# chaiyujin/sdfa-2019

Measured on AMD Instinct MI355X. Metric: animation frames/s/node (10 s@16 kHz clips); max|Δdgrad| vs CPU ref, higher is better.
Workload: dtype f32

## Files before the change

### sdfa-2019_amd/csrc/api_core.cpp

```cpp
#include "../../include/sdfa_stream.h"
#include "host.h"

#include <climits>
#include <cstdio>
#include <cstring>
#include <string>

static thread_local std::string g_err;

int sdfa_failv(int code, const char *fmt, va_list ap) {
    char buf[512];
    vsnprintf(buf, sizeof buf, fmt, ap);
    g_err = buf;
    return code;
}

int sdfa_fail(int code, const char *fmt, ...) {
    va_list ap;
    va_start(ap, fmt);
    sdfa_failv(code, fmt, ap);
    va_end(ap);
    return code;
}

thread_local int g_sdfa_mel_fft_radix4 = 0;
thread_local int g_sdfa_gather_plain_order = 0;
thread_local int g_sdfa_frontend_two_kernel = 0;
thread_local int g_sdfa_frontend_stream_block = 0;
thread_local int g_sdfa_frontend_stream_slots = 0;
thread_local int g_sdfa_frontend_stream_spin_max = 0;
thread_local int g_sdfa_frontend_stream_phases = 0;
thread_local int g_sdfa_frontend_t_major = 0;
extern thread_local int g_sdfa_gemm_variant;
thread_local int g_sdfa_freq_lstm_shape = 0;
thread_local int g_sdfa_pca_lds = 0;
thread_local int g_sdfa_pca_fp32 = 0;
thread_local int g_sdfa_conv_fp32 = 0;
thread_local int g_sdfa_time_lstm_split = 0;
thread_local int g_sdfa_time_lstm_fuse_x = 0;
thread_local int g_sdfa_time_lstm_handoff = 0;
thread_local int g_sdfa_time_lstm_timeout_us = 0;
thread_local int g_sdfa_share_gx0_off = 0;
thread_local int g_sdfa_encoder_dedup_off = 0;
thread_local int g_sdfa_share_hash_bits = 0;
thread_local int g_sdfa_freq_proj_tail = 0;
thread_local int g_sdfa_attn_unfused = 0;

extern "C" {

int sdfa_abi_version(void) { return SDFA_ABI_VERSION; }
int sdfa_stream_abi_version(void) { return SDFA_STREAM_ABI_VERSION; }
const char *sdfa_last_error(void) { return g_err.c_str(); }

int sdfa_debug_set_option(const char *name, int value) {
    struct Option { const char *name; int *var; int lo = INT_MIN, hi = INT_MAX; const char *accepts = nullptr; };
    thread_local const Option options[] = {
        {"attn_unfused", &g_sdfa_attn_unfused},
        {"share_gx0_off", &g_sdfa_share_gx0_off},
        {"encoder_dedup_off", &g_sdfa_encoder_dedup_off},
        {"share_hash_bits", &g_sdfa_share_hash_bits, 0, 32, "0 (the whole hash) or 1..32 low bits"},
        {"freq_proj_tail", &g_sdfa_freq_proj_tail, 0, 2, "0 (rule), 1 (never) or 2 (always)"},
        {"frontend_two_kernel", &g_sdfa_frontend_two_kernel},
        {"frontend_stream_phases", &g_sdfa_frontend_stream_phases},
        {"frontend_stream_spin_max", &g_sdfa_frontend_stream_spin_max, 0, INT_MAX, "0 (default) or a positive poll count"},
        {"frontend_stream_block", &g_sdfa_frontend_stream_block, 0, 256, "0 (default) or 1..256 frames"},
        {"frontend_stream_slots", &g_sdfa_frontend_stream_slots, 0, 256, "0 (default) or 1..256 workgroups per block"},
        {"gather_plain_order", &g_sdfa_gather_plain_order},
        {"mel_fft_radix4", &g_sdfa_mel_fft_radix4},
        {"frontend_t_major", &g_sdfa_frontend_t_major},
        {"time_lstm_timeout_us", &g_sdfa_time_lstm_timeout_us},
        {"time_lstm_handoff", &g_sdfa_time_lstm_handoff},
        {"time_lstm_split", &g_sdfa_time_lstm_split},
        {"time_lstm_fuse_x", &g_sdfa_time_lstm_fuse_x, 0, 3, "0 (rule), 1 (never), 2 or 3 (always, 32- / 64-frame tiles)"},
        {"gemm_variant", &g_sdfa_gemm_variant},
        {"freq_lstm_shape", &g_sdfa_freq_lstm_shape},
        {"pca_lds", &g_sdfa_pca_lds},
        {"conv_fp32", &g_sdfa_conv_fp32},
        {"pca_fp32", &g_sdfa_pca_fp32},
    };
    for (const Option &o : options)
        if (name && !strcmp(name, o.name)) {
            if (value < o.lo || value > o.hi) return sdfa_fail(SDFA_EINVAL, "%s: %s", o.name, o.accepts);
            *o.var = value;
            return SDFA_OK;
        }
    return sdfa_fail(SDFA_EINVAL, "unknown option '%s'", name ? name : "(null)");
}

}
```

### sdfa-2019_amd/csrc/api_forward.cpp

```cpp
#include "common.h"
#include "host.h"
#include "kernels.h"
#include "model.h"

#include <algorithm>

extern thread_local int g_sdfa_gemm_variant, g_sdfa_freq_lstm_shape, g_sdfa_pca_lds, g_sdfa_pca_fp32, g_sdfa_conv_fp32, g_sdfa_share_gx0_off, g_sdfa_attn_unfused, g_sdfa_encoder_dedup_off,
    g_sdfa_freq_proj_tail, g_sdfa_share_hash_bits;

namespace {

constexpr int64_t CT_WORDS = 2048, CT_FLAGS = 16, ST_WORDS = SDFA_WS_STATUS_BYTES / 4;

struct Ws {
    int64_t P1, X3, HF, Z, GX, H0, H1, KP, QC, QP, ZK, SH, ZU, total;
    int64_t TRUNK, A0, A1, COEF;
    int64_t CT_FREQ, CT_PCA, CT_FLAG;
};

Ws layout(int64_t Nc, bool keep) {
    const int64_t Mc = 64 * Nc;
    Ws w{};
    int64_t o = 0;
    auto take = [&](int64_t n) { int64_t r = o; o += round_up(n, 64); return r; };
    take(ST_WORDS);
    if (keep) {
        w.P1 = take(2048 * Mc); w.X3 = take(2048 * Mc); w.HF = take((int64_t)HF_SLAB_ROWS * 4 * Mc); w.Z = take(256 * Mc);
        w.GX = take(2048 * Mc); w.H0 = take(512 * Mc); w.H1 = take(512 * Mc); w.KP = take(128 * Mc);
    } else {
        const int64_t A = take(2048 * Mc);
        const int64_t B = take(2048 * Mc);
        w.HF = take((int64_t)HF_SLAB_ROWS * 4 * Mc);
        w.P1 = A; w.GX = A;
        w.X3 = B; w.Z = B; w.H0 = B + 256 * Mc; w.H1 = B + 768 * Mc; w.KP = B + 1280 * Mc;
    }
    w.QC = take(512 * Nc); w.QP = take(128 * Nc); w.ZK = take(512 * Nc);
    const int64_t R = take(2560 * Nc);
    w.TRUNK = R; w.A0 = R + 512 * Nc; w.A1 = R + 1024 * Nc; w.COEF = R + 1280 * Nc;
    w.SH = take(sdfa_share_table_words(Nc) + 111);
    w.ZU = keep ? take(256 * Mc) : w.P1;
    const int64_t CT = take(CT_WORDS);
    w.CT_FREQ = CT; w.CT_PCA = CT + 1; w.CT_FLAG = CT + CT_FLAGS;
    w.total = o;
    return w;
}

int64_t capacity(int64_t bytes, bool keep) {
    const int64_t per128 = layout(128, keep).total * 4;
    int64_t nc = (bytes / per128 + 2) * 128;
    while (nc > 0 && layout(nc, keep).total * 4 > bytes) nc -= 128;
    return nc;
}

struct Prof {
    const sdfa_model *m;
    hipStream_t s;
    hipEvent_t pending = nullptr;
    void begin(const char *stage) {
        if (!m->profile) return;
        sdfa_model::Ev e; e.stage = stage;
        (void)hipEventCreate(&e.a); (void)hipEventCreate(&e.b);
// ... 64 lines not shown
    case SDFA_PREC_BF16X3_ATTENTION: return stage == STAGE_ATTENTION ? 3 : 0;
    case SDFA_PREC_BF16X6: return 6;
    case SDFA_PREC_BF16X3: return 3;
    case SDFA_PREC_BF16: return 1;
    default: return 0;
    }
}

int sdfa_model_set_precision(sdfa_model *m, int mode) {
    if (!m) return sdfa_fail(SDFA_EINVAL, "null model");
    if (mode < SDFA_PREC_FP32 || mode > SDFA_PREC_BF16X6) return sdfa_fail(SDFA_EINVAL, "unknown precision mode %d", mode);
    m->precision = mode;
    return SDFA_OK;
}

int sdfa_model_precision(const sdfa_model *m) { return m ? m->precision : SDFA_EINVAL; }

int sdfa_model_set_reserved_cus(sdfa_model *m, int k) {
    if (!m) return sdfa_fail(SDFA_EINVAL, "null model");
    if (k < 0 || k > 128) return sdfa_fail(SDFA_EINVAL, "reserved_cus must be in [0, 128], got %d", k);
    m->reserved_cus.store(k);
    return SDFA_OK;
}

static int encoder_impl(const sdfa_model *m, const float *d_audio_feat, int64_t n_frames, const int32_t *d_frame_clip,
                        const int64_t *d_frame_start, int hop, float *d_z, float *d_align, void *d_workspace,
                        int64_t workspace_bytes, void *stream) {
    if (!m || !m->finalized) return sdfa_fail(SDFA_ESTATE, "encoder_forward: model not finalised");
    if (n_frames == 0) return SDFA_OK;
    if (!d_audio_feat || !d_z || !d_workspace || n_frames < 0) return sdfa_fail(SDFA_EINVAL, "encoder_forward: bad argument");
    if (((uintptr_t)d_workspace | (uintptr_t)d_audio_feat | (uintptr_t)d_z) & 15) return sdfa_fail(SDFA_EINVAL, "encoder_forward: pointers must be 16-byte aligned");
    if ((uintptr_t)d_align & 3) return sdfa_fail(SDFA_EINVAL, "encoder_forward: d_align must be 4-byte aligned");
    const int64_t cap = capacity(workspace_bytes, m->keep);
    if (cap < 128) return sdfa_fail(SDFA_ENOSPACE, "encoder_forward: workspace of %lld bytes holds no 128-frame chunk", (long long)workspace_bytes);
    hipStream_t s = (hipStream_t)stream;
    Prof pf{m, s};
    float *ws = (float *)d_workspace;
    for (int64_t f0 = 0; f0 < n_frames; f0 += cap) {
        const int64_t N = std::min(cap, n_frames - f0);
        const int64_t Nc = round_up(N, 128), Mc = 64 * Nc;
        const Ws w = layout(Nc, m->keep);
        ConvArgs ca{};
        ca.audio_feat = d_audio_feat + f0 * (64 * 128 * 3); ca.N = N; ca.Nc = Nc; ca.Mc = Mc;
        ca.w1 = m->w1; ca.b1 = m->b1; ca.s1 = m->s1; ca.t1 = m->t1; ca.P1 = ws + w.P1;
        ca.w2 = m->w2; ca.b2 = m->b2; ca.s2 = m->s2; ca.t2 = m->t2;
        ca.w3 = m->w3; ca.b3 = m->b3; ca.s3 = m->s3; ca.t3 = m->t3; ca.X3 = ws + w.X3;
        const bool table = d_frame_clip != nullptr;
        const bool share = table || (!m->keep && !g_sdfa_encoder_dedup_off);
        const int64_t *d_ulimit = nullptr;
        int32_t *col_to_u = nullptr;
        bool split_tail = false;
        int64_t fat_grid = 0;
        const int64_t *d_qfull = nullptr;
        if (share) {
            ShareArgs sa{};
            sa.N = N; sa.Nc = Nc; sa.Mc = Mc;
            sdfa_share_carve(sa, reinterpret_cast<int32_t *>(ws + w.SH));
            split_tail = !m->keep && stage_terms(m, STAGE_BODY) == 0 && g_sdfa_gemm_variant == 0 && Mc / 256 >= 512 && g_sdfa_freq_proj_tail != 1;
            if (split_tail) {
                fat_grid = sdfa_fat_grid(256, Mc, sdfa_cu_count(), m->reserved_cus.load());
                sa.fat_grid = (int)fat_grid; sa.tail_mode = g_sdfa_freq_proj_tail;
            }
            pf.begin("share_map");
            if (table) {
                sa.frame_clip = d_frame_clip + f0; sa.frame_start = d_frame_start + f0; sa.hop = hop;
                sa.t_lo = 6; sa.t_hi = 58;
                HIP_TRY(sdfa_launch_share_map(sa, s));
            } else {
                sa.feat = ca.audio_feat;
                sa.hash = reinterpret_cast<uint64_t *>(ws + w.HF);
                sa.group_slots = sdfa_share_group_slots(N);
                sa.group_key = sa.hash + Mc; sa.group_first = reinterpret_cast<uint32_t *>(sa.group_key + sa.group_slots);
                sa.hash_bits = g_sdfa_share_hash_bits;
                HIP_TRY(sdfa_launch_share_map_content(sa, s));
            }
            pf.end();
            d_ulimit = sa.counts + 1; d_qfull = sa.counts + 2; col_to_u = sa.col_to_u;
            ca.col_src = sa.col_src; ca.col_limit = d_ulimit;
        }
        const int conv_terms = g_sdfa_conv_fp32 ? 0 : stage_terms(m, STAGE_BODY);
        if (m->keep && conv_terms) {
            pf.begin("conv1"); HIP_TRY(sdfa_launch_conv1(ca, s)); pf.end();
            ca.wb = m->cv_wb; ca.terms = conv_terms;
            pf.begin("conv23"); HIP_TRY(sdfa_launch_conv123(ca, s)); pf.end();
        } else if (m->keep) {
            pf.begin("conv1"); HIP_TRY(sdfa_launch_conv1(ca, s)); pf.end();
            pf.begin("conv23"); HIP_TRY(sdfa_launch_conv23(ca, s)); pf.end();
        } else {
            ca.wb = m->cv_wb; ca.terms = conv_terms;
            pf.begin("conv23"); HIP_TRY(sdfa_launch_conv123(ca, s)); pf.end();
        }

        const int fl_terms = stage_terms(m, STAGE_BODY);
        FreqLstmArgs fa{ws + w.X3, m->fl_w, m->fl_b, ws + w.HF, Mc, d_ulimit, m->fl_wb, fl_terms, reinterpret_cast<int *>(ws + w.CT_FREQ),
                        g_sdfa_freq_lstm_shape ? g_sdfa_freq_lstm_shape : (fl_terms ? 0 : m->freq_shape.load()), m->reserved_cus.load()};
        pf.begin("freq_lstm"); HIP_TRY(sdfa_launch_freq_lstm(fa, s)); pf.end();

        GemmArgs g = sdfa_gemm_k4(m->fp_w, 256, ws + w.HF, Mc, ws + w.Z, Mc, 8192);
        g.bias = m->fp_b; g.q_tile_major = 1; g.q_slab_rows = HF_SLAB_ROWS;
        g.terms = stage_terms(m, STAGE_BODY);
        g.reserve_cus = m->reserved_cus.load();
        if (share) { g.D = ws + w.ZU; g.q_limit = split_tail ? d_qfull : d_ulimit; }
        pf.begin("freq_proj");
        HIP_TRY(sdfa_launch_gemm(g, s));
        if (split_tail) {
            GemmTailArgs gt{m->fp_w, ws + w.HF, m->fp_b, ws + w.ZU, Mc, HF_SLAB_ROWS, d_qfull, d_ulimit, (int)fat_grid - 1};
            HIP_TRY(sdfa_launch_gemm_tail(gt, s));
        }
        pf.end();
        const bool share_gx0 = share && !m->keep && stage_terms(m, STAGE_BODY) == 0 && !g_sdfa_share_gx0_off;
        if (share && !share_gx0) {
            pf.begin("share_expand"); HIP_TRY(sdfa_launch_expand_cols(ws + w.ZU, col_to_u, ws + w.Z, 64, Mc, s)); pf.end();
        }

        const float *xin = share_gx0 ? ws + w.ZU : ws + w.Z;
        float *hout[2] = {ws + w.H0, ws + w.H1};
        const char *gxn[2] = {"gx0", "gx1"}, *lsn[2] = {"lstm0", "lstm1"};
        for (int l = 0; l < 2; ++l) {
            const bool mapped = share_gx0 && l == 0;
            float *gx = mapped ? ws + w.HF : ws + w.GX;
            GemmArgs gi = sdfa_gemm_k4(m->gx_w[l], 2048, xin, Mc, gx, Mc, l == 0 ? 256 : 512);
            gi.terms = stage_terms(m, STAGE_BODY);
            gi.reserve_cus = m->reserved_cus.load();
            if (mapped) gi.q_limit = d_ulimit;
            TimeLstmArgs ta{gx, m->tl_w[l], hout[l], Nc, Mc, m->tl_wb[l], stage_terms(m, STAGE_BODY),
                            reinterpret_cast<unsigned *>(ws + w.CT_FLAG), CT_WORDS - CT_FLAGS, m->tl_w16[l],
                            reinterpret_cast<unsigned *>(ws), m->reserved_cus.load(), mapped ? col_to_u : nullptr};
            if (l == 1 && !m->keep) { ta.X = xin; ta.Wxh = m->tl_wxh1; }
            pf.begin(gxn[l]);
            if (!sdfa_time_lstm_fuses_x(ta)) HIP_TRY(sdfa_launch_gemm(gi, s));
            pf.end();
            pf.begin(lsn[l]); HIP_TRY(sdfa_launch_time_lstm(ta, s)); pf.end();
            xin = hout[l];
        }
        const int at_terms = stage_terms(m, STAGE_ATTENTION);
        const bool key_fused = g_sdfa_attn_unfused != 1;
        pf.begin("attn_proj");
        GemmArgs gk = sdfa_gemm_k4(m->kp_w, 128, ws + w.H1, Mc, ws + w.KP, Mc, 512);
        gk.terms = at_terms;
        if (!key_fused) HIP_TRY(sdfa_launch_gemm(gk, s));
        GemmArgs gc = sdfa_gemm_k4(m->qc_w, 512, ws + w.H1 + 31 * Nc * 4, Mc, ws + w.QC, Nc, 1536);
        gc.seg_k = 512; gc.seg_col = Nc; gc.terms = at_terms;
        HIP_TRY(sdfa_launch_gemm(gc, s));
        GemmArgs gq = sdfa_gemm_k4(m->qp_w, 128, ws + w.QC, Nc, ws + w.QP, Nc, 512);
        gq.terms = at_terms;
        HIP_TRY(sdfa_launch_gemm(gq, s));
        const bool tail_fused = key_fused && (at_terms == 0 || at_terms == 6) && g_sdfa_attn_unfused != 2 && sdfa_attn_fuses_tail(Nc, m->reserved_cus.load());
        if (key_fused) {
            AttnKeyArgs ak{};
// ... 239 lines not shown
```

### sdfa-2019_amd/csrc/kernels.h

```cpp
#pragma once
#include <hip/hip_runtime.h>
#include <stdint.h>

enum { ACT_NONE = 0, ACT_LRELU = 1, ACT_TANH = 2 };

constexpr int HF_SLAB_ROWS = 2048;
enum { OUT_K4 = 0, OUT_ROW = 1 };
constexpr int SDFA_MAX_DESTS = 8;

struct GemmArgs {
    const float *P;
    const float *Q;
    float *D;
    const float *bias;
    const float *cond_w;
    const int64_t *cond_idx;
    int64_t ldp, ldq, ldd;
    int64_t Ppad, Qpad;
    int64_t Pstore;
    int64_t Qreal;
    int K;
    int seg_k;
    int64_t seg_col;
    int act, out_mode, bias_on_q;
// ... 35 lines not shown
    const float *hamm;
    const float2 *twiddle;
    const int *mel_bin0;
    const float *mel_w8;
    int win, hop, sliding, nbins_used, nnz;
};
hipError_t sdfa_launch_frontend(const FrontendConsts &c, const float *pcm, const int64_t *clip_off,
                                const int64_t *clip_len, const int32_t *frame_clip, const int64_t *frame_start,
                                int64_t n_frames, float *audio_feat, hipStream_t s);
hipError_t sdfa_launch_mel_columns(const FrontendConsts &c, const float *pcm, const int64_t *clip_off, const int64_t *clip_len,
                                   const int32_t *frame_clip, const int64_t *frame_start, const int32_t *col_src,
                                   const int64_t *n_distinct, float *mel_table, hipStream_t s);
hipError_t sdfa_launch_mel_stream(const FrontendConsts &c, const float *pcm, const int64_t *clip_off, const int64_t *clip_len,
                                  const int32_t *frame_clip, const int64_t *frame_start, const int32_t *prev, const int32_t *shift,
                                  int64_t n_frames, int block, int slots, int producer_consumer, int spin_max, int *status, float *audio_feat, hipStream_t s);
hipError_t sdfa_launch_mel_ring(const FrontendConsts &c, const float *rings, int r, int n_rings, const int64_t *view_ring, const int64_t *view_hi,
                                const int32_t *frame_view, const int64_t *frame_start, const int32_t *prev, const int32_t *shift, int64_t n_frames,
                                int block, int slots, int producer_consumer, int spin_max, int *status, float *audio_feat, hipStream_t s);
hipError_t sdfa_launch_ring_append(float *rings, int r, int n_rings, const int64_t *seg, int n_seg, const float *src, int64_t n_src, hipStream_t s);
hipError_t sdfa_launch_gather_features(const float *mel_table, const int32_t *col_to_u, int64_t n_frames, int64_t Nc, int frame_major,
                                       float *audio_feat, hipStream_t s);

struct ConvArgs {
    const float *audio_feat;
    int64_t N, Nc, Mc;
    const float *w1, *b1, *s1, *t1;
    float *P1;
    const float *w2, *b2, *s2, *t2;
    const float *w3, *b3, *s3, *t3;
    float *X3;
    const int32_t *col_src;
    const int64_t *col_limit;
    const void *wb;
    int terms;
};
hipError_t sdfa_launch_conv1(const ConvArgs &a, hipStream_t s);
hipError_t sdfa_launch_conv23(const ConvArgs &a, hipStream_t s);
hipError_t sdfa_launch_conv123(const ConvArgs &a, hipStream_t s);

struct FreqLstmArgs {
    const float *X3;
    const float *W;
    const float *bias;
    float *HF;
    int64_t Mc;
    const int64_t *col_limit;
    const void *Wb;
    int terms;
    int *tile_counter;
    int shape;
    int reserve_cus;
};
hipError_t sdfa_launch_freq_lstm(const FreqLstmArgs &a, hipStream_t s);

struct TimeLstmArgs {
    const float *GX;
    const float *W;
    float *H;
    int64_t Nc, Mc;
    const void *Wb;
    int terms;
    unsigned *flags;
    int64_t flag_words;
    const float *W16;
    unsigned *status;
    int reserve_cus;
    const int32_t *col_map;
    const float *X = nullptr;
    const float *Wxh = nullptr;
};
hipError_t sdfa_launch_time_lstm(const TimeLstmArgs &a, hipStream_t s);
int sdfa_time_lstm_fuses_x(const TimeLstmArgs &a);

struct AttnArgs {
    const float *KP;
    const float *QP;
    const float *H;
    const float *v;
    const float *b;
    float *Zk4;
    float *z_out;
    float *align_out;
    int64_t N, Nc, Mc;
    const float *S;
};
hipError_t sdfa_launch_attn(const AttnArgs &a, hipStream_t s);

struct AttnKeyArgs {
    const float *Wk;
    const float *H;
    const float *QP;
    const float *v, *b;
    float *S;
    int64_t Nc, Mc;
    int terms;
    int reserve_cus;
    int ts_shift;
    int fuse_tail;
    float *Zk4, *z_out, *align_out;
    int64_t N;
};
bool sdfa_attn_fuses_tail(int64_t Nc, int reserve_cus);
hipError_t sdfa_launch_attn_key_score(const AttnKeyArgs &a, hipStream_t s);

hipError_t sdfa_launch_rows_to_k4(const float *src, int64_t N, int F, float *dst, int64_t ld, hipStream_t s);
hipError_t sdfa_launch_rows_seg_to_k4(const float *src, int64_t src_ld, int64_t N, int c0, int nf, float *dst, int64_t ld,
                                      int f0, int nf_pad, hipStream_t s);
hipError_t sdfa_launch_k4_to_rows(const float *src, int64_t ld, int64_t N, int F, int f0, int nf, float *dst,
                                  int64_t dst_ld, hipStream_t s);
hipError_t sdfa_launch_tap(const float *src, int what, int64_t N, int64_t Nc, float *dst, hipStream_t s);

struct ShareArgs {
    const int32_t *frame_clip;
    const int64_t *frame_start;
    int hop;
    int t_lo, t_hi;
    int frame_major;
    int64_t N, Nc, Mc;
    int32_t *prev, *shift;
    int32_t *owner, *flag, *uid;
    int32_t *tile_sum;
    int32_t *col_src;
    int32_t *col_to_u;
    int64_t *counts;
    const float *feat;
    uint64_t *hash;
    uint64_t *group_key;
    uint32_t *group_first;
    int64_t group_slots;
    int hash_bits;
    int fat_grid;
    int tail_mode;
};
inline int64_t sdfa_share_table_words(int64_t Nc) { return 16 + 2 * Nc + 5 * (64 * Nc) + (64 * Nc) / 1024 + 1; }
inline int64_t sdfa_share_group_slots(int64_t N) { int64_t s = 1024; while (s < 2 * 64 * N) s <<= 1; return s; }
inline void sdfa_share_carve(ShareArgs &a, int32_t *base) {
    a.counts = reinterpret_cast<int64_t *>(base);
    a.prev = base + 16; a.shift = a.prev + a.Nc;
    a.owner = a.shift + a.Nc; a.flag = a.owner + a.Mc; a.uid = a.flag + a.Mc;
    a.col_src = a.uid + a.Mc; a.col_to_u = a.col_src + a.Mc; a.tile_sum = a.col_to_u + a.Mc;
}
hipError_t sdfa_launch_share_map(const ShareArgs &a, hipStream_t s);
hipError_t sdfa_launch_share_map_content(const ShareArgs &a, hipStream_t s);
hipError_t sdfa_launch_share_prev(const ShareArgs &a, hipStream_t s);
hipError_t sdfa_launch_expand_cols(const float *Zu, const int32_t *col_to_u, float *Z, int nquads, int64_t Mc, hipStream_t s);

struct GemmTailArgs {
    const float *P, *Q, *bias;
    float *D;
    int64_t ldd;
    int q_slab_rows;
    const int64_t *q_lo, *q_hi;
    int max_tiles;
};
hipError_t sdfa_launch_gemm_tail(const GemmTailArgs &a, hipStream_t s);
inline int64_t sdfa_fat_grid(int64_t rows, int64_t cols, int cus, int reserve_cus) {
    const int64_t ntiles = (rows / 256) * (cols / 256), wgs = cus - reserve_cus > 1 ? cus - reserve_cus : 1;
    return ntiles < wgs ? ntiles : wgs;
}

struct MeshArgs {
    const float *dgrad;
    int64_t n_frames;
    int n_tris, n_verts, n_free, free_pad;
    int n_src_tris;
    const int64_t *seek_src;
    const float *seek_w;
    const float *reg_xt;
    const int *inc_ptr;
    const int *inc_tri;
    const float *inc_coef;
    const int *vert_col;
    const float *tmpl;
    float *rhs;
    const float *sol;
    float *verts;
    int64_t ld;
};
hipError_t sdfa_launch_mesh_rhs(const MeshArgs &a, hipStream_t s);
hipError_t sdfa_launch_mesh_scatter(const MeshArgs &a, hipStream_t s);
hipError_t sdfa_launch_seek_plan(const int32_t *tslist, const int64_t *frame_off, const int64_t *query_off, int n_clips, double fps,
                                 int64_t n_queries, int64_t *src, float *w, hipStream_t s);
hipError_t sdfa_launch_seek_rows(const float *rows, int64_t width, const int64_t *src, const float *w, int64_t nq, float *out, hipStream_t s);
struct DgradArgs {
    const float *src;
    const float *target;
    const uint32_t *faces;
    const uint8_t *mask;
    int64_t n_frames;
    int n_tris, n_verts, target_is_offsets;
// ... 38 lines not shown
```

### sdfa-2019_amd/csrc/lstm.hip

```cpp
#include "common.h"
#include "kernels.h"

namespace {

typedef float f32x2 __attribute__((ext_vector_type(2)));
typedef float f32x4n __attribute__((ext_vector_type(4)));

__device__ __forceinline__ f32x2 rcp2(f32x2 d) { return f32x2{__builtin_amdgcn_rcpf(d.x), __builtin_amdgcn_rcpf(d.y)}; }
__device__ __forceinline__ f32x2 exp2n(f32x2 y) { return f32x2{__builtin_amdgcn_exp2f(-y.x), __builtin_amdgcn_exp2f(-y.y)}; }

__device__ __forceinline__ f32x2 sigmoid2(f32x2 x) {
    return rcp2(exp2n(x * 1.4426950408889634f) + 1.0f);
}

__device__ __forceinline__ f32x2 tanh2(f32x2 x) {
    const f32x2 y = x * 2.8853900817779268f;
    const f32x2 e = {__builtin_amdgcn_exp2f(-__builtin_fabsf(y.x)), __builtin_amdgcn_exp2f(-__builtin_fabsf(y.y))};
    const f32x2 t = (1.0f - e) * rcp2(1.0f + e);
    return f32x2{__builtin_copysignf(t.x, x.x), __builtin_copysignf(t.y, x.y)};
}

template <bool FREQ = false>
__device__ __forceinline__ void lstm_cell_quad(const f32x16 &ai, const f32x16 &af, const f32x16 &ag, const f32x16 &ao,
                                               f32x16 &c, int g, float4 &hq) {
    f32x2 hv[2];
#pragma unroll
    for (int p = 0; p < 2; ++p) {
        const int r = 4 * g + 2 * p;
        f32x2 cp = {c[r], c[r + 1]};
        if (FREQ) {
            constexpr float K2 = 2.8853900817779268f;
            const f32x2 ig = rcp2(exp2n(f32x2{ai[r], ai[r + 1]}) + 1.0f);
            const f32x2 fg = rcp2(exp2n(f32x2{af[r], af[r + 1]}) + 1.0f);
            const f32x2 fc = fg * cp;
            const f32x2 gg = __builtin_elementwise_fma(rcp2(exp2n(f32x2{ag[r], ag[r + 1]}) + 1.0f), f32x2{2.0f * K2, 2.0f * K2}, f32x2{-K2, -K2});
            const f32x2 cn = __builtin_elementwise_fma(ig, gg, fc);
            c[r] = cn.x; c[r + 1] = cn.y;
            const f32x2 eo = exp2n(f32x2{ao[r], ao[r + 1]}), ec = exp2n(cn);
            hv[p] = (1.0f - ec) * rcp2((1.0f + eo) * (1.0f + ec));
            continue;
        }
        const f32x2 ig = sigmoid2(f32x2{ai[r], ai[r + 1]});
        const f32x2 fg = sigmoid2(f32x2{af[r], af[r + 1]});
        const f32x2 fc = fg * cp;
        {
            const f32x2 gg = tanh2(f32x2{ag[r], ag[r + 1]});
            const f32x2 og = sigmoid2(f32x2{ao[r], ao[r + 1]});
            const f32x2 cn = __builtin_elementwise_fma(ig, gg, fc);
            c[r] = cn.x; c[r + 1] = cn.y;
            hv[p] = og * tanh2(cn);
        }
    }
    hq = make_float4(hv[0].x, hv[0].y, hv[1].x, hv[1].y);
}


template <bool SHARED, bool PERSIST>
__global__ __launch_bounds__(256, 2) void freq_lstm_v2_kernel(FreqLstmArgs a) {
    constexpr int NJ = 2, BT = 64;
    __shared__ float4 sH[32][BT];
    __shared__ float4 sX[2][16][BT];
    __shared__ float sBias[512];
    __shared__ int sTile;

    const int tid = threadIdx.x, lane = tid & 63, wave = tid >> 6;
    const int l31 = lane & 31, h = lane >> 5;
    const float4 *__restrict__ X3 = reinterpret_cast<const float4 *>(a.X3);
    float4 *__restrict__ HF = reinterpret_cast<float4 *>(a.HF);
    const int n_tiles = (int)(a.Mc / BT) * 2;
  for (;;) {
    int dir;
    int64_t m0;
    if (PERSIST) {
        if (tid == 0) sTile = atomicAdd(a.tile_counter, 1);
        __syncthreads();
        const int t = __builtin_amdgcn_readfirstlane(sTile);
        if (t >= n_tiles) break;
        dir = t & 1;
        m0 = (int64_t)(t >> 1) * BT;
        if (SHARED && m0 >= *a.col_limit) break;
    } else {
        dir = (blockIdx.x >> 3) & 1;
        m0 = (int64_t)(((blockIdx.x >> 4) << 3) | (blockIdx.x & 7)) * BT;
        if (SHARED && m0 >= *a.col_limit) return;
    }
    const float4 *__restrict__ W = reinterpret_cast<const float4 *>(a.W) + (size_t)dir * 48 * 512;

    sBias[tid] = a.bias[dir * 512 + tid];
    sBias[256 + tid] = a.bias[dir * 512 + 256 + tid];

    const float4 *__restrict__ xsrc = X3 + (int64_t)wave * a.Mc + m0 + lane;
#define XDMA(f, buf)                                                                                                   \
    _Pragma("unroll") for (int i = 0; i < 4; ++i)                                                                      \
        __builtin_amdgcn_global_load_lds((const void __attribute__((address_space(1))) *)(xsrc + (int64_t)((f)*16 + 4 * i) * a.Mc), \
                                         (void __attribute__((address_space(3))) *)(&sX[buf][4 * i + wave][0]), 16, 0, 0);
    XDMA(dir ? 31 : 0, 0)

    f32x16 c[NJ];
#pragma unroll
    for (int j = 0; j < NJ; ++j)
#pragma unroll
        for (int r = 0; r < 16; ++r) c[j][r] = 0.f;

    typedef unsigned int u32x4 __attribute__((ext_vector_type(4)));
    const unsigned long long wptr = (unsigned long long)(W + wave * 128);
    const unsigned long long wuni = ((unsigned long long)(unsigned)__builtin_amdgcn_readfirstlane((int)(wptr >> 32)) << 32) |
                                    (unsigned long long)(unsigned)__builtin_amdgcn_readfirstlane((int)(unsigned)wptr);
// ... 1800 lines not shown
```

### sdfa-2019_amd/csrc/share.hip

```cpp
#include "common.h"
#include "kernels.h"

namespace {


__global__ void share_prev_kernel(ShareArgs a) {
    const int64_t n = (int64_t)blockIdx.x * blockDim.x + threadIdx.x;
    if (n >= a.Nc) return;
    int prev = -1, shift = 0;
    if (n < a.N) {
        const int clip = a.frame_clip[n];
        const int64_t s = a.frame_start[n];
        for (int back = 1; back <= 64 && n - back >= 0; ++back) {
            const int64_t q = n - back;
            if (a.frame_clip[q] != clip) break;
            const int64_t diff = s - a.frame_start[q];
            if (diff <= 0) break;
            if (diff > (int64_t)(a.t_hi - a.t_lo) * a.hop) break;
            if (diff % a.hop == 0) { prev = (int)q; shift = (int)(diff / a.hop); break; }
        }
    }
    a.prev[n] = prev;
    a.shift[n] = shift;
}
// ... 98 lines not shown
    }
    const uint64_t bad = __ballot(differ) >> (32 * half) & 0xffffffffull;
    if (l == 0) {
        const int64_t o = bad ? i : cand;
        a.owner[i] = (int)o;
        a.flag[i] = o == i ? 1 : 0;
    }
}

__device__ __forceinline__ int block_inclusive_scan_1024(int v, int *part) {
    const int tid = threadIdx.x;
    part[tid] = v;
    __syncthreads();
    for (int off = 1; off < 1024; off <<= 1) {
        const int x = tid >= off ? part[tid - off] : 0;
        __syncthreads();
        part[tid] += x;
        __syncthreads();
    }
    return part[tid];
}

__global__ __launch_bounds__(1024) void share_scan_tiles_kernel(ShareArgs a) {
    __shared__ int part[1024];
    const int64_t i = (int64_t)blockIdx.x * 1024 + threadIdx.x;
    const int f = i < a.Mc ? a.flag[i] : 0;
    const int inc = block_inclusive_scan_1024(f, part);
    if (i < a.Mc) a.uid[i] = inc - f;
    if (threadIdx.x == 1023) a.tile_sum[blockIdx.x] = inc;
}

constexpr int TAIL_NUM = 3, TAIL_DEN = 4;
__global__ __launch_bounds__(1024) void share_scan_sums_kernel(ShareArgs a, int ntiles) {
    __shared__ int part[1024];
    int carry = 0;
    for (int base = 0; base < ntiles; base += 1024) {
        const int t = base + threadIdx.x;
        const int v = t < ntiles ? a.tile_sum[t] : 0;
        const int inc = block_inclusive_scan_1024(v, part);
        if (t < ntiles) a.tile_sum[t] = carry + inc - v;
        carry += part[1023];
        __syncthreads();
    }
    if (threadIdx.x == 0) {
        const int64_t mu = carry, pad = (mu + 255) / 256 * 256;
        a.counts[0] = mu;
        a.counts[1] = pad;
        int64_t q_full = pad;
        if (a.fat_grid > 0 && a.tail_mode != 1) {
            const int64_t T = pad / 256, G = a.fat_grid, r = T % G;
            if (a.tail_mode == 2 || r * TAIL_DEN <= G * TAIL_NUM) q_full = (T - r) * 256;
        }
        a.counts[2] = q_full;
    }
}

__global__ __launch_bounds__(1024) void share_scan_fix_kernel(ShareArgs a) {
    const int64_t i = (int64_t)blockIdx.x * 1024 + threadIdx.x;
    const int64_t mu = a.counts[0], pad = a.counts[1];
    if (i < a.Mc) {
        const int u = a.uid[i] + a.tile_sum[blockIdx.x];
        a.uid[i] = u;
        int64_t n;
        int t;
        col_of(a, i, n, t);
        if (a.flag[i]) a.col_src[u] = (int)(n * 64 + t);
    }
    if (i >= mu && i < pad) a.col_src[i] = -1;
}

__global__ void share_assign_kernel(ShareArgs a) {
    const int64_t m = (int64_t)blockIdx.x * blockDim.x + threadIdx.x;
    if (m >= a.Mc) return;
    const int o = a.owner[m];
    a.col_to_u[m] = o >= 0 ? a.uid[o] : 0;
}

__global__ void expand_cols_kernel(const float4 *__restrict__ Zu, const int32_t *__restrict__ col_to_u, float4 *__restrict__ Z,
                                   int nquads, int64_t Mc) {
    const int64_t m = (int64_t)blockIdx.x * blockDim.x + threadIdx.x;
    if (m >= Mc) return;
    const int64_t u = col_to_u[m];
    for (int q = 0; q < nquads; ++q) Z[(int64_t)q * Mc + m] = Zu[(int64_t)q * Mc + u];
}

}

static void launch_share_numbering(const ShareArgs &a, hipStream_t s) {
    const int ntiles = (int)((a.Mc + 1023) / 1024);
    hipLaunchKernelGGL(share_scan_tiles_kernel, dim3(ntiles), dim3(1024), 0, s, a);
    hipLaunchKernelGGL(share_scan_sums_kernel, dim3(1), dim3(1024), 0, s, a, ntiles);
    hipLaunchKernelGGL(share_scan_fix_kernel, dim3(ntiles), dim3(1024), 0, s, a);
    hipLaunchKernelGGL(share_assign_kernel, dim3((unsigned)((a.Mc + 255) / 256)), dim3(256), 0, s, a);
}

hipError_t sdfa_launch_share_map_content(const ShareArgs &a, hipStream_t s) {
    const hipError_t e = hipMemsetAsync(a.group_key, 0xff, (size_t)a.group_slots * 12, s);
    if (e != hipSuccess) return e;
    hipLaunchKernelGGL(share_hash_kernel, dim3((unsigned)(a.N * 8)), dim3(256), 0, s, a);
    hipLaunchKernelGGL(share_resolve_kernel, dim3((unsigned)(a.Nc * 8)), dim3(256), 0, s, a);
    launch_share_numbering(a, s);
    return hipGetLastError();
}

hipError_t sdfa_launch_share_map(const ShareArgs &a, hipStream_t s) {
    hipLaunchKernelGGL(share_prev_kernel, dim3((unsigned)((a.Nc + 255) / 256)), dim3(256), 0, s, a);
// ... 16 lines not shown
```

Measured before the change: 151,600.

## Split freq LSTM wave-quantization tail into a finer-grained 32-column tail kernel

The share-map scan now computes a cutoff column count so the main frequency LSTM processes only whole waves of 64-column tiles across the CUs. A new persistent tail kernel then handles the leftover columns in 32-column tiles, pulled from an atomic work queue. This targets the final partial wave where most CUs would sit idle. In exchange it adds an extra kernel launch and a duplicated hand-scheduled MFMA LSTM loop, and moves the shared cell math into a header.

```diff
diff --git a/sdfa-2019_amd/csrc/api_core.cpp b/sdfa-2019_amd/csrc/api_core.cpp
--- a/sdfa-2019_amd/csrc/api_core.cpp
+++ b/sdfa-2019_amd/csrc/api_core.cpp
@@ -44,6 +44,7 @@
 thread_local int g_sdfa_encoder_dedup_off = 0;
 thread_local int g_sdfa_share_hash_bits = 0;
 thread_local int g_sdfa_freq_proj_tail = 0;
+thread_local int g_sdfa_freq_lstm_tail = 0;
 thread_local int g_sdfa_attn_unfused = 0;
 
 extern "C" {
@@ -60,6 +61,7 @@
         {"encoder_dedup_off", &g_sdfa_encoder_dedup_off},
         {"share_hash_bits", &g_sdfa_share_hash_bits, 0, 32, "0 (the whole hash) or 1..32 low bits"},
         {"freq_proj_tail", &g_sdfa_freq_proj_tail, 0, 2, "0 (rule), 1 (never) or 2 (always)"},
+        {"freq_lstm_tail", &g_sdfa_freq_lstm_tail, 0, 2, "0 (rule), 1 (never) or 2 (always)"},
         {"frontend_two_kernel", &g_sdfa_frontend_two_kernel},
         {"frontend_stream_phases", &g_sdfa_frontend_stream_phases},
         {"frontend_stream_spin_max", &g_sdfa_frontend_stream_spin_max, 0, INT_MAX, "0 (default) or a positive poll count"},
diff --git a/sdfa-2019_amd/csrc/api_forward.cpp b/sdfa-2019_amd/csrc/api_forward.cpp
--- a/sdfa-2019_amd/csrc/api_forward.cpp
+++ b/sdfa-2019_amd/csrc/api_forward.cpp
@@ -6,7 +6,7 @@
 #include <algorithm>
 
 extern thread_local int g_sdfa_gemm_variant, g_sdfa_freq_lstm_shape, g_sdfa_pca_lds, g_sdfa_pca_fp32, g_sdfa_conv_fp32, g_sdfa_share_gx0_off, g_sdfa_attn_unfused, g_sdfa_encoder_dedup_off,
-    g_sdfa_freq_proj_tail, g_sdfa_share_hash_bits;
+    g_sdfa_freq_proj_tail, g_sdfa_freq_lstm_tail, g_sdfa_share_hash_bits;
 
 namespace {
 
@@ -177,6 +177,11 @@
         bool split_tail = false;
         int64_t fat_grid = 0;
         const int64_t *d_qfull = nullptr;
+        const int fl_terms = stage_terms(m, STAGE_BODY);
+        const int fl_shape = g_sdfa_freq_lstm_shape ? g_sdfa_freq_lstm_shape : (fl_terms ? 0 : m->freq_shape.load());
+        const bool freq_tail = share && !m->keep && fl_terms == 0 && fl_shape != 5 && fl_shape != 3 && g_sdfa_freq_lstm_tail != 1;
+        const int64_t *d_cfull = nullptr;
+        int *d_fqueue = nullptr;
         if (share) {
             ShareArgs sa{};
             sa.N = N; sa.Nc = Nc; sa.Mc = Mc;
@@ -186,6 +191,7 @@
                 fat_grid = sdfa_fat_grid(256, Mc, sdfa_cu_count(), m->reserved_cus.load());
                 sa.fat_grid = (int)fat_grid; sa.tail_mode = g_sdfa_freq_proj_tail;
             }
+            if (freq_tail) { sa.freq_grid = sdfa_freq_grid(sdfa_cu_count(), m->reserved_cus.load()); sa.freq_tail_mode = g_sdfa_freq_lstm_tail; }
             pf.begin("share_map");
             if (table) {
                 sa.frame_clip = d_frame_clip + f0; sa.frame_start = d_frame_start + f0; sa.hop = hop;
@@ -200,7 +206,7 @@
                 HIP_TRY(sdfa_launch_share_map_content(sa, s));
             }
             pf.end();
-            d_ulimit = sa.counts + 1; d_qfull = sa.counts + 2; col_to_u = sa.col_to_u;
+            d_ulimit = sa.counts + 1; d_qfull = sa.counts + 2; d_cfull = sa.counts + 3; d_fqueue = sa.freq_queue; col_to_u = sa.col_to_u;
             ca.col_src = sa.col_src; ca.col_limit = d_ulimit;
         }
         const int conv_terms = g_sdfa_conv_fp32 ? 0 : stage_terms(m, STAGE_BODY);
@@ -216,10 +222,15 @@
             pf.begin("conv23"); HIP_TRY(sdfa_launch_conv123(ca, s)); pf.end();
         }
 
-        const int fl_terms = stage_terms(m, STAGE_BODY);
-        FreqLstmArgs fa{ws + w.X3, m->fl_w, m->fl_b, ws + w.HF, Mc, d_ulimit, m->fl_wb, fl_terms, reinterpret_cast<int *>(ws + w.CT_FREQ),
-                        g_sdfa_freq_lstm_shape ? g_sdfa_freq_lstm_shape : (fl_terms ? 0 : m->freq_shape.load()), m->reserved_cus.load()};
-        pf.begin("freq_lstm"); HIP_TRY(sdfa_launch_freq_lstm(fa, s)); pf.end();
+        FreqLstmArgs fa{ws + w.X3, m->fl_w, m->fl_b, ws + w.HF, Mc, freq_tail ? d_cfull : d_ulimit, m->fl_wb, fl_terms, reinterpret_cast<int *>(ws + w.CT_FREQ),
+                        fl_shape, m->reserved_cus.load()};
+        pf.begin("freq_lstm");
+        HIP_TRY(sdfa_launch_freq_lstm(fa, s));
+        if (freq_tail) {
+            FreqLstmTailArgs ft{ws + w.X3, m->fl_w, m->fl_b, ws + w.HF, Mc, d_cfull, d_ulimit, d_fqueue, m->reserved_cus.load()};
+            HIP_TRY(sdfa_launch_freq_lstm_tail(ft, s));
+        }
+        pf.end();
 
         GemmArgs g = sdfa_gemm_k4(m->fp_w, 256, ws + w.HF, Mc, ws + w.Z, Mc, 8192);
         g.bias = m->fp_b; g.q_tile_major = 1; g.q_slab_rows = HF_SLAB_ROWS;
diff --git a/sdfa-2019_amd/csrc/freq_tail.hip b/sdfa-2019_amd/csrc/freq_tail.hip
--- /dev/null
+++ b/sdfa-2019_amd/csrc/freq_tail.hip
@@ -0,0 +1,135 @@
+#include "common.h"
+#include "kernels.h"
+#include "lstm_cell.h"
+
+namespace {
+
+__global__ __launch_bounds__(256, 2) void freq_lstm_tail_kernel(FreqLstmTailArgs a) {
+    constexpr int BT = 32, ROWS = 48;
+    extern __shared__ float4 sDynT[];
+    float4 (*sXH)[ROWS][BT] = reinterpret_cast<float4 (*)[ROWS][BT]>(sDynT);
+    float *sBias = reinterpret_cast<float *>(sDynT + 2 * ROWS * BT);
+    int *sTile = reinterpret_cast<int *>(sBias + 512);
+
+    const int tid = threadIdx.x, lane = tid & 63;
+    const int wave = __builtin_amdgcn_readfirstlane(tid >> 6);
+    const int l31 = lane & 31, h = lane >> 5;
+    const float4 *__restrict__ X3 = reinterpret_cast<const float4 *>(a.X3);
+    float4 *__restrict__ HF = reinterpret_cast<float4 *>(a.HF);
+    const int64_t lo = *a.col_lo, hi = std::min<int64_t>(*a.col_hi, a.Mc);
+    typedef unsigned int u32x4 __attribute__((ext_vector_type(4)));
+    for (;;) {
+        if (tid == 0) *sTile = atomicAdd(a.queue, 1);
+        __syncthreads();
+        const int t = __builtin_amdgcn_readfirstlane(*sTile);
+        const int dir = t & 1;
+        const int64_t m0 = lo + (int64_t)(t >> 1) * BT;
+        if (lo < 0 || m0 >= hi) break;
+        const float4 *__restrict__ W = reinterpret_cast<const float4 *>(a.W) + (size_t)dir * 48 * 512;
+        sBias[tid] = a.bias[dir * 512 + tid];
+        sBias[256 + tid] = a.bias[dir * 512 + 256 + tid];
+
+        const float4 *__restrict__ xsrc = X3 + (int64_t)(2 * wave + h) * a.Mc + m0 + l31;
+#pragma unroll
+        for (int i = 0; i < 2; ++i)
+            __builtin_amdgcn_global_load_lds((const void __attribute__((address_space(1))) *)(xsrc + (int64_t)((dir ? 31 : 0) * 16 + 8 * i) * a.Mc),
+                                             (void __attribute__((address_space(3))) *)(&sXH[0][8 * i + 2 * wave][0]), 16, 0, 0);
+
+        f32x16 c;
+#pragma unroll
+        for (int r = 0; r < 16; ++r) c[r] = 0.f;
+
+        const unsigned long long wptr = (unsigned long long)(W + wave * 128);
+        const __amdgpu_buffer_rsrc_t wrs = __builtin_amdgcn_make_buffer_rsrc((void *)wptr, 0, 48 * 512 * 16, 0x00020000);
+        const unsigned woff = (unsigned)((l31 + h * 512) * 16);
+#define FT_W(so, g_) __builtin_bit_cast(float4, (u32x4)__builtin_amdgcn_raw_buffer_load_b128(wrs, woff + 512 * (g_), so, 0))
+#define FT_SB() __builtin_amdgcn_sched_barrier(0);
+#define FT_Q(W0, W1, W2, W3, B, q)                                                                          \
+    {                                                                                                        \
+        acc[0] = MFMA(f4c(W0, q), f4c(B, q), acc[0]);                                                        \
+        acc[1] = MFMA(f4c(W1, q), f4c(B, q), acc[1]);                                                        \
+        acc[2] = MFMA(f4c(W2, q), f4c(B, q), acc[2]);                                                        \
+        acc[3] = MFMA(f4c(W3, q), f4c(B, q), acc[3]);                                                        \
+    }
+#define FT_KB(CW0, CW1, CW2, CW3, CB, NW0, NW1, NW2, NW3, NB, so, bp)                                        \
+    {                                                                                                        \
+        FT_SB() NW0 = FT_W(so, 0); NW1 = FT_W(so, 1); FT_SB()                                                \
+        FT_Q(CW0, CW1, CW2, CW3, CB, 0)                                                                      \
+        FT_SB() NW2 = FT_W(so, 2); NW3 = FT_W(so, 3); FT_SB()                                                \
+        FT_Q(CW0, CW1, CW2, CW3, CB, 1)                                                                      \
+        FT_SB() NB = (bp)[0]; FT_SB()                                                                        \
+        FT_Q(CW0, CW1, CW2, CW3, CB, 2)                                                                      \
+        FT_SB()                                                                                              \
+        FT_Q(CW0, CW1, CW2, CW3, CB, 3)                                                                      \
+    }
+        float4 wa0, wa1, wa2, wa3, wb0, wb1, wb2, wb3, ba, bb;
+        wa0 = FT_W(0u, 0); wa1 = FT_W(0u, 1); wa2 = FT_W(0u, 2); wa3 = FT_W(0u, 3);
+        __syncthreads();
+
+        for (int s = 0; s < 32; ++s) {
+            const int f = dir ? 31 - s : s;
+            const int cur = s & 1;
+            f32x16 acc[4];
+            const float4 *brow = &sXH[cur][h][l31];
+            ba = brow[0];
+            FT_SB()
+#pragma unroll
+            for (int gt = 0; gt < 4; ++gt)
+#pragma unroll
+                for (int g = 0; g < 4; ++g) {
+                    const float4 b = *reinterpret_cast<const float4 *>(&sBias[wave * 128 + gt * 32 + 8 * g + 4 * h]);
+                    acc[gt][4 * g + 0] = b.x; acc[gt][4 * g + 1] = b.y;
+                    acc[gt][4 * g + 2] = b.z; acc[gt][4 * g + 3] = b.w;
+                }
+            const int trips = s > 0 ? 3 : 1;
+#pragma unroll 1
+            for (int t_ = 0; t_ < trips; ++t_) {
+                const float4 *bt = brow + t_ * 16 * BT;
+                const float4 *bn = t_ + 1 < trips ? bt + 16 * BT : brow;
+                const unsigned so = (unsigned)t_ * (8 * 1024 * 16);
+                const unsigned son = t_ + 1 < trips ? so + 8 * 1024 * 16 : 0u;
+                FT_KB(wa0, wa1, wa2, wa3, ba, wb0, wb1, wb2, wb3, bb, so + 1 * 1024 * 16, bt + 1 * 2 * BT)
+                FT_KB(wb0, wb1, wb2, wb3, bb, wa0, wa1, wa2, wa3, ba, so + 2 * 1024 * 16, bt + 2 * 2 * BT)
+                FT_KB(wa0, wa1, wa2, wa3, ba, wb0, wb1, wb2, wb3, bb, so + 3 * 1024 * 16, bt + 3 * 2 * BT)
+                FT_KB(wb0, wb1, wb2, wb3, bb, wa0, wa1, wa2, wa3, ba, so + 4 * 1024 * 16, bt + 4 * 2 * BT)
+                FT_KB(wa0, wa1, wa2, wa3, ba, wb0, wb1, wb2, wb3, bb, so + 5 * 1024 * 16, bt + 5 * 2 * BT)
+                FT_KB(wb0, wb1, wb2, wb3, bb, wa0, wa1, wa2, wa3, ba, so + 6 * 1024 * 16, bt + 6 * 2 * BT)
+                FT_KB(wa0, wa1, wa2, wa3, ba, wb0, wb1, wb2, wb3, bb, so + 7 * 1024 * 16, bt + 7 * 2 * BT)
+                FT_KB(wb0, wb1, wb2, wb3, bb, wa0, wa1, wa2, wa3, ba, son, bn)
+            }
+            FT_SB()
+            float4 xr0, xr1;
+            {
+                const int fn = s + 1 < 32 ? (dir ? 30 - s : s + 1) : f;
+                const float4 *xs = xsrc + (int64_t)(fn * 16) * a.Mc;
+                xr0 = xs[0]; xr1 = xs[8 * a.Mc];
+            }
+#pragma unroll
+            for (int g = 0; g < 4; ++g) {
+                float4 hq;
+                lstm_cell_quad<true>(acc[0], acc[1], acc[2], acc[3], c, g, hq);
+                const int hq_idx = 8 * wave + 2 * g + h;
+                sXH[cur ^ 1][16 + hq_idx][l31] = hq;
+                HF[((m0 >> 7) * (int64_t)HF_SLAB_ROWS + (f * 64 + dir * 32 + hq_idx)) * 128 + (m0 & 127) + l31] = hq;
+            }
+            sXH[cur ^ 1][2 * wave + h][l31] = xr0; sXH[cur ^ 1][8 + 2 * wave + h][l31] = xr1;
+            asm volatile("s_waitcnt lgkmcnt(0)\n\ts_barrier" ::: "memory");
+        }
+#undef FT_W
+#undef FT_SB
+#undef FT_Q
+#undef FT_KB
+    }
+}
+
+}
+
+hipError_t sdfa_launch_freq_lstm_tail(const FreqLstmTailArgs &a, hipStream_t s) {
+    if (!a.X3 || !a.W || !a.bias || !a.HF || !a.col_lo || !a.col_hi || !a.queue || a.Mc <= 0 || a.Mc % 256) return hipErrorInvalidValue;
+    const size_t lds = 2 * 48 * 64 * sizeof(float4) + 512 * sizeof(float) + 16;
+    const hipError_t e = hipFuncSetAttribute(reinterpret_cast<const void *>(freq_lstm_tail_kernel), hipFuncAttributeMaxDynamicSharedMemorySize, (int)lds);
+    if (e != hipSuccess) return e;
+    const int grid = std::max(1, sdfa_cu_count() - a.reserve_cus);
+    hipLaunchKernelGGL(freq_lstm_tail_kernel, dim3((unsigned)grid), dim3(256), lds, s, a);
+    return hipGetLastError();
+}
diff --git a/sdfa-2019_amd/csrc/kernels.h b/sdfa-2019_amd/csrc/kernels.h
--- a/sdfa-2019_amd/csrc/kernels.h
+++ b/sdfa-2019_amd/csrc/kernels.h
@@ -111,6 +111,17 @@
     int reserve_cus;
 };
 hipError_t sdfa_launch_freq_lstm(const FreqLstmArgs &a, hipStream_t s);
+
+struct FreqLstmTailArgs {
+    const float *X3, *W, *bias;
+    float *HF;
+    int64_t Mc;
+    const int64_t *col_lo, *col_hi;
+    int *queue;
+    int reserve_cus;
+};
+hipError_t sdfa_launch_freq_lstm_tail(const FreqLstmTailArgs &a, hipStream_t s);
+inline int sdfa_freq_grid(int cus, int reserve_cus) { return cus - reserve_cus > 1 ? cus - reserve_cus : 1; }
 
 struct TimeLstmArgs {
     const float *GX;
@@ -190,11 +201,15 @@
     int hash_bits;
     int fat_grid;
     int tail_mode;
+    int freq_grid;
+    int freq_tail_mode;
+    int32_t *freq_queue;
 };
 inline int64_t sdfa_share_table_words(int64_t Nc) { return 16 + 2 * Nc + 5 * (64 * Nc) + (64 * Nc) / 1024 + 1; }
 inline int64_t sdfa_share_group_slots(int64_t N) { int64_t s = 1024; while (s < 2 * 64 * N) s <<= 1; return s; }
 inline void sdfa_share_carve(ShareArgs &a, int32_t *base) {
     a.counts = reinterpret_cast<int64_t *>(base);
+    a.freq_queue = base + 10;
     a.prev = base + 16; a.shift = a.prev + a.Nc;
     a.owner = a.shift + a.Nc; a.flag = a.owner + a.Mc; a.uid = a.flag + a.Mc;
     a.col_src = a.uid + a.Mc; a.col_to_u = a.col_src + a.Mc; a.tile_sum = a.col_to_u + a.Mc;
diff --git a/sdfa-2019_amd/csrc/lstm.hip b/sdfa-2019_amd/csrc/lstm.hip
--- a/sdfa-2019_amd/csrc/lstm.hip
+++ b/sdfa-2019_amd/csrc/lstm.hip
@@ -1,58 +1,8 @@
 #include "common.h"
 #include "kernels.h"
+#include "lstm_cell.h"
 
 namespace {
-
-typedef float f32x2 __attribute__((ext_vector_type(2)));
-typedef float f32x4n __attribute__((ext_vector_type(4)));
-
-__device__ __forceinline__ f32x2 rcp2(f32x2 d) { return f32x2{__builtin_amdgcn_rcpf(d.x), __builtin_amdgcn_rcpf(d.y)}; }
-__device__ __forceinline__ f32x2 exp2n(f32x2 y) { return f32x2{__builtin_amdgcn_exp2f(-y.x), __builtin_amdgcn_exp2f(-y.y)}; }
-
-__device__ __forceinline__ f32x2 sigmoid2(f32x2 x) {
-    return rcp2(exp2n(x * 1.4426950408889634f) + 1.0f);
-}
-
-__device__ __forceinline__ f32x2 tanh2(f32x2 x) {
-    const f32x2 y = x * 2.8853900817779268f;
-    const f32x2 e = {__builtin_amdgcn_exp2f(-__builtin_fabsf(y.x)), __builtin_amdgcn_exp2f(-__builtin_fabsf(y.y))};
-    const f32x2 t = (1.0f - e) * rcp2(1.0f + e);
-    return f32x2{__builtin_copysignf(t.x, x.x), __builtin_copysignf(t.y, x.y)};
-}
-
-template <bool FREQ = false>
-__device__ __forceinline__ void lstm_cell_quad(const f32x16 &ai, const f32x16 &af, const f32x16 &ag, const f32x16 &ao,
-                                               f32x16 &c, int g, float4 &hq) {
-    f32x2 hv[2];
-#pragma unroll
-    for (int p = 0; p < 2; ++p) {
-        const int r = 4 * g + 2 * p;
-        f32x2 cp = {c[r], c[r + 1]};
-        if (FREQ) {
-            constexpr float K2 = 2.8853900817779268f;
-            const f32x2 ig = rcp2(exp2n(f32x2{ai[r], ai[r + 1]}) + 1.0f);
-            const f32x2 fg = rcp2(exp2n(f32x2{af[r], af[r + 1]}) + 1.0f);
-            const f32x2 fc = fg * cp;
-            const f32x2 gg = __builtin_elementwise_fma(rcp2(exp2n(f32x2{ag[r], ag[r + 1]}) + 1.0f), f32x2{2.0f * K2, 2.0f * K2}, f32x2{-K2, -K2});
-            const f32x2 cn = __builtin_elementwise_fma(ig, gg, fc);
-            c[r] = cn.x; c[r + 1] = cn.y;
-            const f32x2 eo = exp2n(f32x2{ao[r], ao[r + 1]}), ec = exp2n(cn);
-            hv[p] = (1.0f - ec) * rcp2((1.0f + eo) * (1.0f + ec));
-            continue;
-        }
-        const f32x2 ig = sigmoid2(f32x2{ai[r], ai[r + 1]});
-        const f32x2 fg = sigmoid2(f32x2{af[r], af[r + 1]});
-        const f32x2 fc = fg * cp;
-        {
-            const f32x2 gg = tanh2(f32x2{ag[r], ag[r + 1]});
-            const f32x2 og = sigmoid2(f32x2{ao[r], ao[r + 1]});
-            const f32x2 cn = __builtin_elementwise_fma(ig, gg, fc);
-            c[r] = cn.x; c[r + 1] = cn.y;
-            hv[p] = og * tanh2(cn);
-        }
-    }
-    hq = make_float4(hv[0].x, hv[0].y, hv[1].x, hv[1].y);
-}
 
 
 template <bool SHARED, bool PERSIST>
diff --git a/sdfa-2019_amd/csrc/lstm_cell.h b/sdfa-2019_amd/csrc/lstm_cell.h
--- /dev/null
+++ b/sdfa-2019_amd/csrc/lstm_cell.h
@@ -0,0 +1,57 @@
+#pragma once
+#include "common.h"
+
+namespace {
+
+typedef float f32x2 __attribute__((ext_vector_type(2)));
+typedef float f32x4n __attribute__((ext_vector_type(4)));
+
+__device__ __forceinline__ f32x2 rcp2(f32x2 d) { return f32x2{__builtin_amdgcn_rcpf(d.x), __builtin_amdgcn_rcpf(d.y)}; }
+__device__ __forceinline__ f32x2 exp2n(f32x2 y) { return f32x2{__builtin_amdgcn_exp2f(-y.x), __builtin_amdgcn_exp2f(-y.y)}; }
+
+__device__ __forceinline__ f32x2 sigmoid2(f32x2 x) {
+    return rcp2(exp2n(x * 1.4426950408889634f) + 1.0f);
+}
+
+__device__ __forceinline__ f32x2 tanh2(f32x2 x) {
+    const f32x2 y = x * 2.8853900817779268f;
+    const f32x2 e = {__builtin_amdgcn_exp2f(-__builtin_fabsf(y.x)), __builtin_amdgcn_exp2f(-__builtin_fabsf(y.y))};
+    const f32x2 t = (1.0f - e) * rcp2(1.0f + e);
+    return f32x2{__builtin_copysignf(t.x, x.x), __builtin_copysignf(t.y, x.y)};
+}
+
+template <bool FREQ = false>
+__device__ __forceinline__ void lstm_cell_quad(const f32x16 &ai, const f32x16 &af, const f32x16 &ag, const f32x16 &ao,
+                                               f32x16 &c, int g, float4 &hq) {
+    f32x2 hv[2];
+#pragma unroll
+    for (int p = 0; p < 2; ++p) {
+        const int r = 4 * g + 2 * p;
+        f32x2 cp = {c[r], c[r + 1]};
+        if (FREQ) {
+            constexpr float K2 = 2.8853900817779268f;
+            const f32x2 ig = rcp2(exp2n(f32x2{ai[r], ai[r + 1]}) + 1.0f);
+            const f32x2 fg = rcp2(exp2n(f32x2{af[r], af[r + 1]}) + 1.0f);
+            const f32x2 fc = fg * cp;
+            const f32x2 gg = __builtin_elementwise_fma(rcp2(exp2n(f32x2{ag[r], ag[r + 1]}) + 1.0f), f32x2{2.0f * K2, 2.0f * K2}, f32x2{-K2, -K2});
+            const f32x2 cn = __builtin_elementwise_fma(ig, gg, fc);
+            c[r] = cn.x; c[r + 1] = cn.y;
+            const f32x2 eo = exp2n(f32x2{ao[r], ao[r + 1]}), ec = exp2n(cn);
+            hv[p] = (1.0f - ec) * rcp2((1.0f + eo) * (1.0f + ec));
+            continue;
+        }
+        const f32x2 ig = sigmoid2(f32x2{ai[r], ai[r + 1]});
+        const f32x2 fg = sigmoid2(f32x2{af[r], af[r + 1]});
+        const f32x2 fc = fg * cp;
+        {
+            const f32x2 gg = tanh2(f32x2{ag[r], ag[r + 1]});
+            const f32x2 og = sigmoid2(f32x2{ao[r], ao[r + 1]});
+            const f32x2 cn = __builtin_elementwise_fma(ig, gg, fc);
+            c[r] = cn.x; c[r + 1] = cn.y;
+            hv[p] = og * tanh2(cn);
+        }
+    }
+    hq = make_float4(hv[0].x, hv[0].y, hv[1].x, hv[1].y);
+}
+
+}
diff --git a/sdfa-2019_amd/csrc/share.hip b/sdfa-2019_amd/csrc/share.hip
--- a/sdfa-2019_amd/csrc/share.hip
+++ b/sdfa-2019_amd/csrc/share.hip
@@ -174,6 +174,13 @@
             if (a.tail_mode == 2 || r * TAIL_DEN <= G * TAIL_NUM) q_full = (T - r) * 256;
         }
         a.counts[2] = q_full;
+        int64_t c_full = pad;
+        if (a.freq_grid > 0 && a.freq_tail_mode != 1) {
+            const int64_t T = pad / 32, G = a.freq_grid, tiles = (T - T % G) / 2, r2 = T - 2 * tiles;
+            if (a.freq_tail_mode == 2 || 2 * r2 <= G) c_full = tiles * 64;
+        }
+        a.counts[3] = c_full;
+        if (a.freq_queue) *a.freq_queue = 0;
     }
 }
 
```

Result: no change. 151,700, median of 5 (+0.0%).
